# spaceandtimefdn/blitzar

Hardware: NVIDIA H100
Metric: MSM throughput (scalar*point terms/sec), ristretto255, n=2^20 per GPU (higher is better)
Workload: dtype u32 limbs (integer modular arithmetic)

## Files before the change

blitzar_b200/csrc/api.cu:

```cuda
#include <algorithm>
#include <cctype>
#include <cstdint>
#include <cstdio>
#include <cstdlib>
#include <cstring>
#include <condition_variable>
#include <functional>
#include <mutex>
#include <thread>
#include <memory>
#include <string>
#include <vector>

#include "engine_api.cuh"

using namespace b200;

namespace {

struct State {
  bool initialized = false;
  int device = -1;
  cudaStream_t stream = nullptr;
  cudaStream_t copy_stream = nullptr;
// ... 1314 lines not shown
    B200_CUDA(cudaEventDestroy(copied[k]));
  }
}
unsigned b200_multiexp_handle_add_partition_table(struct sxt_multiexp_handle* handle,
                                                  unsigned window_width) {
  const Entry entry("b200_multiexp_handle_add_partition_table");
  return handle_add_partition_table(handle_of(handle), window_width);
}
unsigned b200_multiexp_handle_partition_window(const struct sxt_multiexp_handle* handle) {
  std::lock_guard<std::mutex> lock(g_mutex);
  const HandleSet* hs = handle_of(handle);
  return hs->shards.empty() ? 0u : hs->shards[0]->ptable_w;
}
namespace {
uint64_t check_multi_pairing(unsigned curve_id, const void* out, uint32_t num_products,
                             const uint32_t* lengths, const void* g1, const void* g2) {
  B200_REQUIRE(curve_id == SXT_CURVE_BLS_381 || curve_id == SXT_CURVE_BN_254,
               "pairings are defined for curve ids 1 (bls12-381) and 2 (bn254) only");
  B200_REQUIRE(num_products == 0 || (out != nullptr && lengths != nullptr),
               "out / lengths must not be null");
  uint64_t total = 0;
  for (uint32_t k = 0; k < num_products; ++k)
    total += lengths[k];
  B200_REQUIRE(total < (1ull << 31), "2^31 or more pairs in one call");
  B200_REQUIRE(total == 0 || (g1 != nullptr && g2 != nullptr), "g1 / g2 must not be null");
  return total;
}
}

void b200_multi_pairing(unsigned curve_id, void* out, uint32_t num_products,
                        const uint32_t* lengths, const void* g1, const void* g2) {
  const Entry entry("b200_multi_pairing");
  const uint64_t n = check_multi_pairing(curve_id, out, num_products, lengths, g1, g2);
  if (num_products == 0)
    return;
  cudaStream_t s = g_state.stream;
  const size_t b1 = curve_vtable(curve_id).abi_proj_bytes;
  const size_t b2 = curve_vtable(curve_id == SXT_CURVE_BLS_381 ? B200_CURVE_BLS12_381_G2
                                                               : B200_CURVE_BN254_G2).abi_proj_bytes;
  const size_t gt = curve_id == SXT_CURVE_BLS_381 ? sizeof(b200_bls12_381_gt) : sizeof(b200_bn254_gt);
  DevBuf<unsigned char> d1(n * b1, s), d2(n * b2, s), dout(num_products * gt, s);
  copy_h2d(d1.p, g1, n * b1, s);
  copy_h2d(d2.p, g2, n * b2, s);
  multi_pairing(ctx(), curve_id, dout.p, num_products, lengths, d1.p, d2.p);
  copy_d2h(out, dout.p, num_products * gt, s);
  stream_sync(s);
}
void b200_multi_pairing_device(unsigned curve_id, void* out, uint32_t num_products,
                               const uint32_t* lengths, const void* g1, const void* g2) {
  const Entry entry("b200_multi_pairing_device");
  check_multi_pairing(curve_id, out, num_products, lengths, g1, g2);
  if (num_products == 0)
    return;
  multi_pairing(ctx(), curve_id, out, num_products, lengths, g1, g2);
}
namespace {
void check_points_call(unsigned curve_id, bool pointers_set, uint64_t n) {
  B200_REQUIRE(curve_id >= SXT_CURVE_BLS_381 && curve_id <= B200_CURVE_BN254_G2,
               "point checks are defined for curve ids 1-5 (a ristretto255 encoding is checked by "
               "decoding it)");
  B200_REQUIRE(n == 0 || pointers_set, "valid / points must not be null");
}
uint64_t count_valid(const uint8_t* valid, uint64_t n) {
  uint64_t count = 0;
  for (uint64_t i = 0; i < n; ++i)
    count += valid[i] != 0;
  return count;
}
}

uint64_t b200_check_points(unsigned curve_id, uint8_t* valid, const void* points, uint64_t n) {
  const Entry entry("b200_check_points");
  check_points_call(curve_id, valid != nullptr && points != nullptr, n);
  if (n == 0)
    return 0;
  cudaStream_t s = g_state.stream;
  const size_t bytes = curve_vtable(curve_id).abi_proj_bytes;
  DevBuf<unsigned char> dp(n * bytes, s), dv(n, s);
  copy_h2d(dp.p, points, n * bytes, s);
  check_points(ctx(), curve_id, dv.p, dp.p, n);
  copy_d2h(valid, dv.p, n, s);
  stream_sync(s);
  return count_valid(valid, n);
}
uint64_t b200_decode_points(unsigned curve_id, void* out_p2, uint8_t* valid, const void* encoded,
                            uint64_t n) {
  const Entry entry("b200_decode_points");
  check_points_call(curve_id, out_p2 != nullptr && valid != nullptr && encoded != nullptr, n);
  if (n == 0)
    return 0;
  cudaStream_t s = g_state.stream;
  const CurveVTable& vt = curve_vtable(curve_id);
  DevBuf<unsigned char> de(n * vt.abi_commit_bytes, s), dout(n * vt.abi_proj_bytes, s), dv(n, s);
  copy_h2d(de.p, encoded, n * vt.abi_commit_bytes, s);
  decode_points(ctx(), curve_id, dout.p, dv.p, de.p, n);
  copy_d2h(out_p2, dout.p, n * vt.abi_proj_bytes, s);
  copy_d2h(valid, dv.p, n, s);
  stream_sync(s);
  return count_valid(valid, n);
}
void b200_check_points_device(unsigned curve_id, uint8_t* valid, const void* points, uint64_t n) {
  const Entry entry("b200_check_points_device");
  check_points_call(curve_id, valid != nullptr && points != nullptr, n);
  check_points(ctx(), curve_id, valid, points, n);
}
void b200_decode_points_device(unsigned curve_id, void* out_p2, uint8_t* valid,
                               const void* encoded, uint64_t n) {
  const Entry entry("b200_decode_points_device");
  check_points_call(curve_id, out_p2 != nullptr && valid != nullptr && encoded != nullptr, n);
  decode_points(ctx(), curve_id, out_p2, valid, encoded, n);
}
unsigned b200_selftest_lane_arithmetic(unsigned warps, unsigned seed) {
  const Entry entry("b200_selftest_lane_arithmetic");
  return selftest_lane_arithmetic(ctx(), warps, seed);
}
unsigned b200_field_op(unsigned field, unsigned op, uint64_t n, const uint32_t* a,
                       const uint32_t* b, uint32_t* out) {
  const Entry entry("b200_field_op");
  B200_REQUIRE(n == 0 || (a != nullptr && out != nullptr), "null operand or result array");
  return field_op(ctx(), field, op, n, a, b, out);
}
unsigned b200_selftest_sort(const sxt_sequence_descriptor* columns, unsigned num,
                            unsigned window_bits) {
  const Entry entry("b200_selftest_sort");
  B200_REQUIRE(num == 0 || columns != nullptr, "columns == nullptr");
  B200_REQUIRE(window_bits <= 20, "window_bits in 0..20");
  return selftest_sort(ctx(), columns, num, window_bits);
}
void b200_set_reduce_groups(unsigned g1, unsigned gn) {
  std::lock_guard<std::mutex> lock(g_mutex);
  auto pow2 = [](unsigned v, unsigned dflt) {
    if (v < 2)
      return dflt;
    unsigned p = 2;
    while (p * 2 <= v)
      p *= 2;
    return p;
  };
  g_state.opt.reduce_g1 = pow2(g1, 16u);
  g_state.opt.reduce_gn = pow2(gn, 4u);
}
void b200_profile_accumulate(int enable) {
  std::lock_guard<std::mutex> lock(g_mutex);
  KernelTimer::get().enabled = enable != 0;
}
void b200_profile_read(float* total_ms, unsigned* launches) {
  std::lock_guard<std::mutex> lock(g_mutex);
  KernelTimer::get().read(total_ms, launches);
}
void b200_set_tuning(unsigned window_bits, unsigned chunk1, unsigned chunkn) {
  std::lock_guard<std::mutex> lock(g_mutex);
  g_state.opt.window_bits = window_bits;
  g_state.opt.chunk1 = chunk1;
  g_state.opt.chunkn = chunkn ? chunkn : 8;
}

}
```

blitzar_b200/csrc/engine_api.cuh:

```cuda
#pragma once
#include <algorithm>
#include <cmath>
#include <cstdint>
#include <vector>

#include "../../include/blitzar_b200.h"
#include "runtime.cuh"

namespace b200 {

struct MsmOptions {
  u32 window_bits = 0;
  u32 chunk1 = 0;
  u32 chunkn = 8;
  u32 reduce_g1 = 16;
  u32 reduce_gn = 4;
  u64 quad_threshold = 32768;
  u64 max_group_entries = 1ull << 30;
  u64 max_range_entries = 1ull << 31;
  int pair_levels = -1;
  u32 pair_batch = 0;
  int range_skew = 0;
  u32 uniform_add = 2;
  u32 gens_normalized = 0;
  const u32* unit_veto = nullptr;
  u32 normalize_gens = 1;
  u32 lane_tail = 1;
  u32 scatter_window_major = 0;
  u32 sort_path = 1;
  u32 table_policy = 0;
};

struct EngineCtx {
  stream_t s;
  MsmOptions opt;
  const void* builtin;
  uint64_t num_builtin;
  stream_t tail = stream_t();
  u32 builtin_window_bits = 0, builtin_windows = 0;
  u32 partition_policy = 0;
};

struct Handle {
  unsigned curve_id;
  unsigned n;
  void* gens;
  unsigned window_bits = 0, windows = 1;
  void* ptable = nullptr;
  unsigned ptable_w = 0;
  uint64_t ptable_groups = 0;
};

inline unsigned table_window_bits(uint64_t n, size_t gen_bytes, double budget_bytes) {
  if (n < 1024)
    return 0;
  unsigned best = 0;
  double best_cost = 1e300;
  for (unsigned c = 10; c <= 20; ++c) {
    const double W = 256 / c + 1;
    if (W * (double)n * (double)gen_bytes > budget_bytes || W * (double)n >= 2147483648.0)
      continue;
    const double cost = W * (double)n + 2.5 * (double)(1u << (c - 1));
    if (cost < best_cost) {
      best_cost = cost;
      best = c;
    }
  }
  return best;
}

template <class T> struct DevBuf {
  T* p = nullptr;
  stream_t s;
  DevBuf(size_t count, stream_t s_) : s(s_) { p = (T*)dev_alloc(count * sizeof(T), s); }
  ~DevBuf() { dev_free(p, s); }
  DevBuf(const DevBuf&) = delete;
  DevBuf& operator=(const DevBuf&) = delete;
};

inline uint64_t range_begin(uint64_t n, uint32_t r, uint32_t num_ranges, int skew = 0) {
  if (r == 0)
    return 0;
  if (r >= num_ranges)
    return n;
  if (skew == 0 || n < 64ull * num_ranges)
    return n * r / num_ranges;
  const double t = (double)r / (double)num_ranges;
  const double f = skew > 0 ? 1.0 - (1.0 - t) * std::sqrt(1.0 - t) : t * std::sqrt(t);
  uint64_t b = (uint64_t)((double)n * f);
  const uint64_t lo = r, hi = n - (num_ranges - r);
  return b < lo ? lo : (b > hi ? hi : b);
}
typedef void (*range_wait_fn)(void* user, uint64_t begin, uint64_t end);

inline uint64_t check_descriptors(const sxt_sequence_descriptor* d, uint32_t num) {
  B200_REQUIRE(d != nullptr, "descriptors == nullptr");
  uint64_t longest = 0;
  for (uint32_t i = 0; i < num; ++i) {
    B200_REQUIRE(d[i].n == 0 || d[i].data != nullptr, "descriptor.n > 0 with data == nullptr");
    B200_REQUIRE(d[i].element_nbytes != 0 && d[i].element_nbytes <= 32,
                 "descriptor.element_nbytes must be in 1..32");
    if (d[i].is_signed)
      B200_REQUIRE(d[i].element_nbytes <= 16 &&
                       (d[i].element_nbytes & (d[i].element_nbytes - 1)) == 0,
                   "signed columns need a power-of-two element_nbytes <= 16");
    B200_REQUIRE(d[i].n < (1ull << 31), "column too long");
    longest = longest < d[i].n ? d[i].n : longest;
  }
  return longest;
}

inline uint64_t fixed_row_bytes(int mode, unsigned element_num_bytes, const unsigned* bit_table,
                                unsigned num_outputs) {
  uint64_t row_bits = 0;
  if (mode == 0) {
    B200_REQUIRE(element_num_bytes >= 1 && element_num_bytes <= 32, "element_num_bytes in 1..32");
    row_bits = 8ull * element_num_bytes * num_outputs;
  } else {
    for (unsigned j = 0; j < num_outputs; ++j) {
      B200_REQUIRE(bit_table[j] > 0 && bit_table[j] <= 256, "output bit width must be in 1..256");
      row_bits += bit_table[j];
    }
  }
  return (row_bits + 7) / 8;
}

struct GenLayout {
  struct Piece {
    uint64_t src, pos, count;
  };
  std::vector<Piece> segments;
  std::vector<uint32_t> base;
  uint64_t total = 0;
  uint64_t max_n = 0;

  GenLayout(const sxt_sequence_descriptor* d, uint32_t num, const uint64_t* offsets)
      : base(num, 0), n_(num, 0) {
    std::vector<uint32_t> order;
    for (uint32_t j = 0; j < num; ++j) {
      n_[j] = d[j].n;
      max_n = std::max<uint64_t>(max_n, d[j].n);
      if (d[j].n) {
        B200_REQUIRE(offset(offsets, j) <= ~0ull - d[j].n, "generator offset + column length overflows");
        order.push_back(j);
      }
    }
    std::stable_sort(order.begin(), order.end(), [offsets](uint32_t a, uint32_t b) {
      return offset(offsets, a) < offset(offsets, b);
    });
    for (uint32_t j : order) {
      const uint64_t lo = offset(offsets, j), hi = lo + n_[j];
      if (segments.empty() || lo > segments.back().src + segments.back().count) {
        const uint64_t pos = segments.empty() ? 0 : segments.back().pos + segments.back().count;
        segments.push_back({lo, pos, 0});
      }
      Piece& s = segments.back();
      s.count = std::max(s.count, hi - s.src);
      B200_REQUIRE(s.pos + s.count < (1ull << 31),
                   "merged generator intervals of 2^31 or more generators");
      base[j] = (uint32_t)(s.pos + (lo - s.src));
    }
    total = segments.empty() ? 0 : segments.back().pos + segments.back().count;
  }
  bool within(uint64_t limit) const {
    return segments.empty() || segments.back().src + segments.back().count <= limit;
  }
  std::vector<Piece> needed(uint64_t b, uint64_t e) const {
// ... 177 lines not shown
```

blitzar_b200/csrc/msm.cuh:

```cuda
#pragma once
#include <algorithm>
#include <vector>

#include "batch_affine.cuh"
#include "curve.cuh"
#include "engine_api.cuh"
#include "lanefield.cuh"

namespace b200 {

struct ColumnDesc {
  const unsigned char* base;
  u64 row_stride;
  u32 bit_offset;
  u32 bit_width;
  u32 n;
  u32 is_signed;
  u32 first_window;
  u32 num_windows;
  u32 table_n;
  u32 gen_base;
};
B200_HD u32 bucket_windows(const ColumnDesc& col) { return col.table_n ? (col.num_windows ? 1u : 0u) : col.num_windows; }

// ... 383 lines not shown
    __syncthreads();
    for (u32 i = threadIdx.x; i < size; i += kBlock) {
      const u64 e = stage[i];
      tmp[delta[__ldg(&map[entry_key(e) >> sh])] + i] = e;
    }
  }
};

struct BinSortBody {
  static constexpr int kBlock = 1024;
  static constexpr size_t kSmem = kBinCap * sizeof(u64) + kBinSpan * sizeof(u32);
  const u64* tmp;
  const u32* bin_start;
  const u32* bin_micro;
  const u32* nbins_ptr;
  u32 shift;
  u64 nkeys;
  u64* entries;
  u32* counts;
  __device__ void run(u32 b, unsigned char* smem) const {
    __shared__ u32 ws[32];
    if (b >= *nbins_ptr)
      return;
    u64* sorted = (u64*)smem;
    u32* h = (u32*)(smem + kBinCap * sizeof(u64));
    const u32 lo = bin_start[b], size = bin_start[b + 1] - lo;
    const u64 klo = (u64)bin_micro[b] << shift, khi_m = (u64)bin_micro[b + 1] << shift;
    const u32 span = (u32)((khi_m < nkeys ? khi_m : nkeys) - klo);
    const bool local = size <= kBinCap;
    for (u32 k = threadIdx.x; k < span; k += kBlock)
      h[k] = 0;
    __syncthreads();
#pragma unroll 4
    for (u32 i = threadIdx.x; i < size; i += kBlock)
      atomicAdd(&h[entry_key(tmp[(u64)lo + i]) - (u32)klo], 1u);
    __syncthreads();
    const u32 per = (span + kBlock - 1) / kBlock, k0 = min(threadIdx.x * per, span),
              k1 = min(k0 + per, span);
    u32 sum = 0;
    for (u32 k = k0; k < k1; ++k)
      sum += h[k];
    u32 total;
    u32 run = block_exclusive_scan<kBlock>(sum, ws, &total);
    for (u32 k = k0; k < k1; ++k) {
      const u32 n = h[k];
      h[k] = run;
      run += n;
      counts[klo + k] = lo + run;
    }
    __syncthreads();
    if (!local) {
      for (u32 i = threadIdx.x; i < size; i += kBlock) {
        const u64 e = tmp[(u64)lo + i];
        entries[(u64)lo + atomicAdd(&h[entry_key(e) - (u32)klo], 1u)] = e;
      }
      return;
    }
#pragma unroll 4
    for (u32 i = threadIdx.x; i < size; i += kBlock) {
      const u64 e = tmp[(u64)lo + i];
      sorted[atomicAdd(&h[entry_key(e) - (u32)klo], 1u)] = e;
    }
    __syncthreads();
    for (u32 i = threadIdx.x; i < size; i += kBlock)
      entries[(u64)lo + i] = sorted[i];
  }
};

inline u32 binned_sort_shift(u64 nkeys) {
  u32 shift = 0;
  while ((nkeys + (1ull << shift) - 1) >> shift > kMicroBins)
    ++shift;
  return shift;
}

inline void binned_sort(stream_t s, const ColumnDesc* d_cols, const u64* d_col_start, u32 ncols,
                        u32 c, u32 nbuckets, u64 total_terms, u64 max_entries, u32 max_windows,
                        u64 nkeys, u64* entries, u32* counts, u32* d_m) {
  const u32 shift = binned_sort_shift(nkeys);
  const u32 nmicro = (u32)((nkeys + (1ull << shift) - 1) >> shift);
  const u32 span_micro = std::max(1u, kBinSpan >> shift);
  u32* ws = (u32*)dev_alloc((5ull * nmicro + 3) * sizeof(u32), s);
  u32 *micro_counts = ws, *bin_of = ws + nmicro, *bin_cursor = ws + 2ull * nmicro,
      *bin_start = ws + 3ull * nmicro, *bin_micro = ws + 4ull * nmicro + 1,
      *nbins = ws + 5ull * nmicro + 2;
  u64* tmp = (u64*)dev_alloc(std::max<u64>(max_entries, 1) * sizeof(u64), s);
  dev_zero(micro_counts, nmicro * sizeof(u32), s);
  const u64 count_tile = 4096;
  launch_blocks(MicroCountBody{d_cols, d_col_start, ncols, c, nbuckets, total_terms,
                               (u32)count_tile, shift, nmicro, micro_counts},
                (total_terms + count_tile - 1) / count_tile, nmicro * sizeof(u32), s);
  launch_blocks(PlanBinsBody{micro_counts, nmicro, span_micro, nkeys, bin_of, bin_start, bin_micro,
                             bin_cursor, nbins, counts, d_m},
                1, nmicro * sizeof(u32), s);
  const size_t scatter_smem = 220 * 1024;
  const size_t bin_bytes = (2ull * nmicro + 2) * sizeof(u32);
  const u64 stage_entries = (scatter_smem - bin_bytes) / sizeof(u64);
  u64 scatter_tile = std::max<u64>(1, stage_entries / max_windows);
  if (scatter_tile > (u64)CoarseScatterBody::kBlock)
    scatter_tile -= scatter_tile % CoarseScatterBody::kBlock;
  launch_blocks(CoarseScatterBody{d_cols, d_col_start, ncols, c, nbuckets, total_terms,
                                  (u32)scatter_tile, shift, nmicro, bin_of, nbins, bin_cursor, tmp},
                (total_terms + scatter_tile - 1) / scatter_tile, scatter_smem, s);
  launch_blocks(BinSortBody{tmp, bin_start, bin_micro, nbins, shift, nkeys, entries, counts}, nmicro,
                BinSortBody::kSmem, s);
  dev_free(tmp, s);
  dev_free(ws, s);
}
#endif

template <class C> struct FillIdentityBody {
  static constexpr int kBlock = 256;
  static constexpr u32 kChunks = sizeof(typename C::Point) / 16;
  static_assert(sizeof(typename C::Point) % 16 == 0, "points are made of 16-byte aligned fields");
  uint4* p;
  B200_HD void operator()(u64 t) const {
    const typename C::Point id = C::identity();
    const u32 k = (u32)(t % kChunks);
    uint4 v = ((const uint4*)&id)[0];
#pragma unroll
    for (u32 j = 1; j < kChunks; ++j)
      if (j == k)
        v = ((const uint4*)&id)[j];
    p[t] = v;
  }
};
template <class C> inline void fill_identity(stream_t s, typename C::Point* p, u64 n) {
  launch(FillIdentityBody<C>{(uint4*)p}, n * FillIdentityBody<C>::kChunks, s);
}

struct BucketOffsets {
  const u32* ends;
  const u32* starts;
  B200_HD u32 begin(u64 k) const { return starts ? starts[k] : (k ? ends[k - 1] : 0u); }
  B200_HD u32 end(u64 k) const { return ends[k]; }
};

template <class C> struct MergeBucketsBody {
  static constexpr int kBlock = 128;
  BucketOffsets offsets;
  const typename C::Point* scratch;
  typename C::Point* buckets;
  B200_HD void operator()(u64 k) const {
    if (offsets.begin(k) == offsets.end(k))
      return;
    typename C::Point b = buckets[k];
    C::add(b, b, scratch[k]);
    buckets[k] = b;
  }
};

template <class C, bool kGather, class X = SeqExec, bool kUniform = false, bool kUnitZ = false>
struct AccumulateBody {
  static constexpr int kBlock = 128;
  static constexpr int kMinBlocks = !kGather ? 1 : (C::F::N > 8 ? 2 : 3);
  typedef typename C::Point Point;
  typedef typename C::Gen Gen;
  const u32* keys;
  const u64* entries;
  const Gen* gens;
  const Point* pieces;
  const u32* m_ptr;
  u32 K;
  u32 final_level;
  Point* buckets;
  u32* out_keys;
  Point* out_pieces;
  u32* out_m_ptr;
  const u32* unit_veto;

  B200_HD void close_run(u64 t, u32 key, const Point& acc, bool writer, bool& first_seg) const {
    if (final_level || !first_seg) {
      if (writer)
        buckets[key] = acc;
    } else if (writer) {
      out_keys[2 * t] = key;
      out_pieces[2 * t] = acc;
    }
    first_seg = false;
  }
  template <bool kUnit> B200_HD Gen load_gen(u32 idx) const {
    if constexpr (kUnit)
      return C::load_unit_gen(gens + idx);
    else
      return gens[idx];
  }
  template <bool kUnit>
  B200_HD void gather_walk(u64 t, u64 b, u64 e, bool writer, u32& cur, Point& acc,
                           bool& first_seg) const {
    u64 ent = entries[b];
    Gen g = load_gen<kUnit>(entry_gen(ent));
    cur = entry_key(ent);
    for (u64 i = b; i < e; ++i) {
      u64 ent_n = ent;
      Gen g_n = g;
      if (i + 1 < e) {
        ent_n = entries[i + 1];
        g_n = load_gen<kUnit>(entry_gen(ent_n));
      }
      const u32 k = entry_key(ent);
      const bool negate = entry_negate(ent);
      if (kUniform) {
        if (i == b || k != cur) {
          if (i != b) {
            close_run(t, cur, acc, writer, first_seg);
            cur = k;
          }
          acc = C::identity();
        }
        C::template add_gen<X>(acc, acc, g, negate, kUnit);
      } else {
        const bool start = i == b || k != cur;
        if (k != cur) {
          close_run(t, cur, acc, writer, first_seg);
          cur = k;
        }
        if (start)
          C::gen_to_point(acc, g, negate);
        else
          C::template add_gen<X>(acc, acc, g, negate, kUnit);
      }
      ent = ent_n;
      g = g_n;
    }
  }
  B200_HD void operator()(u64 tid) const {
    const u64 t = tid / X::kLanes;
    const bool writer = (tid % X::kLanes) == 0;
    const u64 M = *m_ptr;
    const u64 T = (M + K - 1) / K;
    if (tid == 0 && out_m_ptr)
      *out_m_ptr = final_level ? 0u : (u32)(2 * T);
    u64 b = t * K;
    if (b >= M)
      return;
    u64 e = b + K < M ? b + K : M;
    u32 cur;
    Point acc;
    bool first_seg = true;
    if constexpr (kGather) {
      if (kUnitZ && unit_veto && *unit_veto)
        gather_walk<false>(t, b, e, writer, cur, acc, first_seg);
      else
        gather_walk<kUnitZ>(t, b, e, writer, cur, acc, first_seg);
    } else {
      cur = keys[b];
      acc = pieces[b];
      for (u64 i = b + 1; i < e; ++i) {
        const u32 k = keys[i];
        if (k == cur) {
          C::template add<X>(acc, acc, pieces[i]);
        } else {
          close_run(t, cur, acc, writer, first_seg);
          cur = k;
          acc = pieces[i];
        }
      }
    }
    if (final_level) {
      close_run(t, cur, acc, writer, first_seg);
      return;
    }
    if (!writer)
      return;
    if (first_seg) {
      close_run(t, cur, acc, writer, first_seg);
      acc = C::identity();
    }
    out_keys[2 * t + 1] = cur;
    out_pieces[2 * t + 1] = acc;
  }
};

struct WindowUsedBody {
  static constexpr int kBlock = 64;
  BucketOffsets offsets;
  u32 nbuckets;
  u32* window_used;
  B200_HD void operator()(u64 w) const {
    if (offsets.begin(w * nbuckets) != offsets.begin((w + 1) * nbuckets))
      window_used[w] = 1u;
  }
};

template <class C, class Ex = SeqExec> struct ReduceBody {
  static constexpr int kBlock = 64;
  typedef typename C::Point Point;
  const Point* X;
  const Point* Cin;
  u32 m_in, g, log2g;
  Point* Xout;
  Point* Cout;
  const u32* window_used;
  u32 nbuckets;
  B200_HD void operator()(u64 tid) const {
    const u64 t = tid / Ex::kLanes;
    const bool writer = (tid % Ex::kLanes) == 0;
    const u32 m_out = m_in / g;
    const u32 w = (u32)(t / m_out), k = (u32)(t % m_out);
    if (window_used[w] == 0) {
      if (writer) {
        Xout[t] = C::identity();
        Cout[t] = C::identity();
      }
      return;
    }
    const Point* x = X + (u64)w * m_in + (u64)k * g;
    Point run = x[g - 1];
    Point acc = Cin ? C::identity() : run;
    if (Cin) {
      acc = run;
      if (g == 1)
        acc = C::identity();
    }
    for (u32 r = g - 1; r-- > 0;) {
      C::template add<Ex>(run, run, x[r]);
      if (r > 0 || !Cin)
        C::template add<Ex>(acc, acc, run);
    }
    if (Cin) {
      const Point* cin = Cin + (u64)w * m_in + (u64)k * g;
      for (u32 r = 0; r < g; ++r)
        C::template add<Ex>(acc, acc, cin[r]);
    }
    for (u32 i = 0; i < log2g; ++i)
      C::template dbl<Ex>(run, run);
    if (writer) {
      Xout[t] = run;
      Cout[t] = acc;
    }
  }
};

template <class C, class X = SeqExec> struct CombineBody {
  static constexpr int kBlock = 32;
  typedef typename C::Point Point;
  const Point* S;
  const ColumnDesc* cols;
  u32 c;
  Point* out;
  B200_HD void operator()(u64 tid) const {
    const u64 j = tid / X::kLanes;
    const bool writer = (tid % X::kLanes) == 0;
    const ColumnDesc col = cols[j];
    if (col.num_windows == 0 || col.n == 0) {
      if (writer)
        out[j] = C::identity();
      return;
    }
    const u32 nw = bucket_windows(col);
    Point acc = S[col.first_window + nw - 1];
    for (u32 w = nw - 1; w-- > 0;) {
      for (u32 i = 0; i < c; ++i)
        C::template dbl<X>(acc, acc);
      C::template add<X>(acc, acc, S[col.first_window + w]);
    }
    if (writer)
      out[j] = acc;
  }
};

#if defined(__CUDACC__) && !defined(B200_EMULATE)
#define B200_LANE_TAIL 1
struct CombineLaneBody {
  static constexpr int kBlock = 32;
  typedef Ed25519 C;
  const C::Point* S;
  const ColumnDesc* cols;
  u32 c;
  C::Point* out;
  __device__ void operator()(u64 tid) const {
    const u64 j = tid >> 5;
    const ColumnDesc col = cols[j];
    if (col.num_windows == 0 || col.n == 0) {
      if ((tid & 31u) == 0)
        out[j] = C::identity();
      return;
    }
    const lane10::Lane L = lane10::lane_info();
    const u32 nw = bucket_windows(col);
    C::Point acc = S[col.first_window + nw - 1];
    for (u32 w = nw - 1; w-- > 0;) {
      u32 t;
      const u32 v = lane10::dbl_n(L, lane10::slice_point(L, acc), (int)c, t);
      lane10::gather_point(acc, v, t);
      C::add<QuadExecConv>(acc, acc, S[col.first_window + w]);
    }
    if ((tid & 31u) == 0)
      out[j] = acc;
  }
};
struct LanePow {
  static __device__ __forceinline__ void pow22523(F25519::E& r, const F25519::E& a) {
    const lane10::Lane L = lane10::lane_info();
    const u32 g = L.base / 10u;
    lane10::gather(r, lane10::pow22523(L, lane10::slice(L, a)), g < 3 ? g : 0u);
  }
};
struct StoreLaneBody {
  static constexpr int kBlock = 32;
  const Ed25519::Point* pts;
  unsigned char* out;
  u64 count;
  __device__ void operator()(u64 tid) const {
    const u32 lane = (u32)tid & 31u, g = lane / 10u;
    const u64 i = (tid >> 5) * 3 + g;
    const bool live = g < 3 && i < count;
    unsigned char enc[32];
    Ed25519::encode<LanePow>(enc, pts[live ? i : count - 1]);
    if (live && lane == 10u * g) {
      uint4* d = (uint4*)(out + 32 * i);
      const uint4* e = (const uint4*)enc;
      d[0] = e[0];
      d[1] = e[1];
    }
  }
};
#endif

template <class C>
inline void launch_store_commit(stream_t s, const typename C::Point* pts, unsigned char* out,
                                u64 count, bool lane_tail = true);

template <class C, bool kProjective> struct IngestBody {
  static constexpr int kBlock = 128;
// ... 395 lines not shown
  p.c = opt.window_bits ? opt.window_bits
                        : choose_window_bits(p.max_n, max_width, p.ncols, point_bytes);
  p.nbuckets = 1u << (p.c - 1);
  u64 max_entries = 0;
  for (auto& col : cols) {
    col.first_window = p.total_windows;
    col.num_windows = col.n ? col.bit_width / p.c + 1 : 0;
    p.total_windows += bucket_windows(col);
    max_entries += (u64)col.n * col.num_windows;
    if (col.table_n)
      B200_REQUIRE((u64)col.table_n * col.num_windows < (1ull << 31), "generator table too large");
    if (col.n)
      B200_REQUIRE((u64)col.gen_base + col.n + (u64)(col.num_windows - 1) * col.table_n < (1ull << 31),
                   "generator index of a column too large");
  }
  p.nkeys = (u64)p.total_windows * p.nbuckets;
  p.total_entries = max_entries;
  B200_REQUIRE(p.nkeys < (1ull << 32), "too many buckets for one pass");
  p.cols = std::move(cols);
  return p;
}

struct StagedRange {
  const ColumnDesc* d_cols = nullptr;
  const u64* d_col_start = nullptr;
  u64 total_terms = 0, max_entries = 0;
  u32 max_windows = 0;
  StagedRange(stream_t s, const MsmPlan& plan, u64 begin, u64 end) {
    const u32 ncols = plan.ncols;
    std::vector<ColumnDesc> cols(plan.cols);
    std::vector<u64> col_start(ncols + 1, 0);
    for (u32 j = 0; j < ncols; ++j) {
      u64 lo = std::min<u64>(begin, cols[j].n), hi = std::min<u64>(end, cols[j].n);
      cols[j].base += lo * cols[j].row_stride;
      cols[j].n = (u32)(hi - lo);
      col_start[j + 1] = col_start[j] + cols[j].n;
      max_entries += (u64)cols[j].n * cols[j].num_windows;
      max_windows = std::max(max_windows, cols[j].n ? cols[j].num_windows : 0u);
    }
    total_terms = col_start[ncols];
    if (total_terms == 0)
      return;
    B200_REQUIRE(max_entries < (1ull << 32) && end - begin < (1ull << 31),
                 "too many (term, window) entries for one sort pass");
    const size_t desc_bytes = ncols * sizeof(ColumnDesc), start_bytes = (ncols + 1) * sizeof(u64);
    std::vector<unsigned char> stage(desc_bytes + start_bytes);
    std::memcpy(stage.data(), cols.data(), desc_bytes);
    std::memcpy(stage.data() + desc_bytes, col_start.data(), start_bytes);
    d_cols = (const ColumnDesc*)stage_to_device(s, stage.data(), stage.size());
    d_col_start = (const u64*)((const unsigned char*)d_cols + desc_bytes);
  }
};

struct SortedLayout {
  u64* entries;
  u32* counts;
  u32* starts;
  u32* d_m;
  u64 slots_max;
  bool binned;
  BucketOffsets offsets() const { return {counts, starts}; }
};

inline SortedLayout sort_entries(stream_t s, const MsmPlan& plan, const StagedRange& r, u32 L,
                                 const MsmOptions& opt, u32* window_used) {
  const u32 ncols = plan.ncols, c = plan.c, nbuckets = plan.nbuckets;
  const u64 nkeys = plan.nkeys, max_entries = r.max_entries, total_terms = r.total_terms;
  SortedLayout out{};
  out.slots_max = L ? ((max_entries + nkeys * ((1ull << L) - 1) + (1ull << L) - 1) >> L) << L : max_entries;
  out.counts = (u32*)dev_alloc((nkeys + 1) * sizeof(u32), s);
  out.d_m = (u32*)dev_alloc(16 * sizeof(u32), s);
  out.entries = (u64*)dev_alloc(out.slots_max * sizeof(u64), s);
#ifdef B200_BINNED_SORT
  out.binned = L == 0 && opt.sort_path != 0 && binned_sort_shift(nkeys) <= kMaxBinShift &&
               (opt.sort_path == 2 || max_entries >= kBinnedSortMinEntries);
  if (out.binned)
    binned_sort(s, r.d_cols, r.d_col_start, ncols, c, nbuckets, total_terms, max_entries,
                r.max_windows, nkeys, out.entries, out.counts, out.d_m);
#endif
  if (!out.binned) {
    dev_zero(out.counts, (nkeys + 1) * sizeof(u32), s);
    launch(CountBody{r.d_cols, r.d_col_start, ncols, c, nbuckets, out.counts}, total_terms, s);
    if (L)
      launch(PadCountsBody{out.counts, (1u << L) - 1u}, nkeys, s);
    exclusive_scan(out.counts, nkeys + 1, s);
    copy_d2d(out.d_m, out.counts + nkeys, sizeof(u32), s);
    if (L) {
      out.starts = (u32*)dev_alloc((nkeys + 1) * sizeof(u32), s);
      copy_d2d(out.starts, out.counts, (nkeys + 1) * sizeof(u32), s);
    }
    const bool window_major = opt.scatter_window_major && r.max_windows > 1;
    launch(ScatterBody{r.d_cols, r.d_col_start, ncols, c, nbuckets, out.counts, out.entries,
                       window_major ? total_terms : 0},
           window_major ? total_terms * r.max_windows : total_terms, s);
  }
  if (L)
    launch(FillPadsBody{out.starts, out.counts, out.entries}, nkeys, s);
  launch(WindowUsedBody{out.offsets(), nbuckets, window_used}, plan.total_windows, s);
  return out;
}

inline unsigned sort_selftest(stream_t s, std::vector<ColumnDesc> cols, u32 c) {
  MsmOptions opt;
  opt.window_bits = c;
  const MsmPlan plan = msm_make_plan(std::move(cols), opt, 160);
  const StagedRange r(s, plan, 0, plan.max_n);
  if (r.total_terms == 0)
    return ~0u;
  const u64 nkeys = plan.nkeys, M = r.max_entries;
  DevBuf<u32> window_used(plan.total_windows, s);
  opt.sort_path = 0;
  const SortedLayout a = sort_entries(s, plan, r, 0, opt, window_used.p);
  opt.sort_path = 2;
  const SortedLayout b = sort_entries(s, plan, r, 0, opt, window_used.p);
  std::vector<u32> ca(nkeys + 1), cb(nkeys + 1), m(1);
  std::vector<u64> ea(M), eb(M);
  copy_d2h(ca.data(), a.counts, (nkeys + 1) * sizeof(u32), s);
  copy_d2h(cb.data(), b.counts, (nkeys + 1) * sizeof(u32), s);
  copy_d2h(m.data(), b.d_m, sizeof(u32), s);
  copy_d2h(ea.data(), a.entries, M * sizeof(u64), s);
  copy_d2h(eb.data(), b.entries, M * sizeof(u64), s);
  stream_sync(s);
  for (void* p : {(void*)a.entries, (void*)a.counts, (void*)a.d_m, (void*)b.entries, (void*)b.counts,
                  (void*)b.d_m, (void*)r.d_cols})
    dev_free(p, s);
  if (!b.binned)
    return ~0u;
  unsigned bad = m[0] == ca[nkeys] ? 0u : 1u;
  for (u64 k = 0; k < nkeys; ++k) {
    const u32 lo = k ? ca[k - 1] : 0u, hi = ca[k];
    if (cb[k] != hi || hi < lo || hi > M) {
      ++bad;
      continue;
    }
    std::sort(ea.begin() + lo, ea.begin() + hi);
    std::sort(eb.begin() + lo, eb.begin() + hi);
    if (!std::equal(ea.begin() + lo, ea.begin() + hi, eb.begin() + lo))
      ++bad;
  }
  return bad;
}

struct RangeHook {
  virtual void before_range(u64 begin, u64 end) = 0;
  virtual void before_accumulate() {}
  virtual ~RangeHook() {}
};

template <class C>
stream_t chunk_walk(stream_t s, stream_t tail, WalkInput<C> walk, u32* d_m, bool unit,
                    const u32* unit_veto, typename C::Point* target, const MsmOptions& opt,
                    std::vector<void*>& to_free) {
  typedef typename C::Point Point;
  u32 K = opt.chunk1 ? std::max(opt.chunk1, 4u) : (walk.m_max >= (1ull << 23) ? 64u : 32u);
  const u32 chunkn = std::max(opt.chunkn, 4u);
  const u32* lvl_keys = nullptr;
  const Point* lvl_pieces = nullptr;
  stream_t cs = s;
  for (int level = 0;; ++level) {
    const bool final_level = walk.m_max <= K;
    u64 T = (walk.m_max + K - 1) / K;
    u32* out_keys = final_level ? nullptr : (u32*)dev_alloc(2 * T * sizeof(u32), cs);
    Point* out_pieces = final_level ? nullptr : (Point*)dev_alloc(2 * T * sizeof(Point), cs);
    to_free.insert(to_free.end(), {out_keys, out_pieces});
    u32* out_m = d_m + 1 + (level % 8);
    const auto launch_level = [&](auto body, u64 threads, stream_t st) {
      body = {lvl_keys, walk.entries, walk.gens, lvl_pieces, walk.m_ptr, K, final_level, target,
              out_keys, out_pieces, out_m, unit_veto};
      launch(body, threads, st);
    };
    if (level == 0) {
      const bool uniform =
          opt.uniform_add == 2 ? C::kCurveId == kRistretto255 : opt.uniform_add != 0;
      constexpr bool kEd = C::kCurveId == kRistretto255;
      const bool unit_path = kEd && unit;
      if (uniform && unit_path)
        launch_level(AccumulateBody<C, true, SeqExec, true, kEd>{}, T, s);
      else if (uniform)
        launch_level(AccumulateBody<C, true, SeqExec, true>{}, T, s);
      else if (unit_path)
        launch_level(AccumulateBody<C, true, SeqExec, false, kEd>{}, T, s);
      else
        launch_level(AccumulateBody<C, true>{}, T, s);
      KernelTimer::get().end(s);
      if (tail != s)
        stream_follow(tail, s);
      cs = tail;
    } else if (T <= opt.quad_threshold) {
      launch_level(AccumulateBody<C, false, QuadExec>{}, T * QuadExec::kLanes, cs);
    } else {
      launch_level(AccumulateBody<C, false>{}, T, cs);
    }
    if (final_level)
      break;
    lvl_keys = out_keys;
    lvl_pieces = out_pieces;
    walk.m_ptr = out_m;
    walk.m_max = 2 * T;
    K = chunkn;
  }
  return cs;
}

template <class C>
void msm_accumulate_range(stream_t s, const MsmPlan& plan, const typename C::Gen* gens, u64 begin,
                          u64 end, bool add_into, typename C::Point* d_buckets,
                          u32* d_window_used, const MsmOptions& opt, stream_t tail,
                          RangeHook* hook = nullptr) {
  const StagedRange r(s, plan, begin, end);
  if (r.total_terms == 0)
    return;
  gens += begin;
  StageRange nvtx_sort("msm: digit count + scan + scatter");
  const u64 max_entries = r.max_entries, nkeys = plan.nkeys;
  u32 L = 0;
  if constexpr (C::kBatchAffine) {
    const double mean = (double)max_entries / (double)nkeys;
    if (opt.pair_levels >= 0)
      L = (u32)opt.pair_levels;
    else if (max_entries >= (1ull << 23))
      while (L < 6 && (double)(32u << L) <= mean)
        ++L;
    while (L > 0 && max_entries + nkeys * ((1ull << L) - 1) >= (1ull << 32) - (1ull << L))
      --L;
  }
  const SortedLayout sorted = sort_entries(s, plan, r, L, opt, d_window_used);
  B200_LOG(3, "range [%llu, %llu): %llu terms, %llu entries max, c=%u, %llu keys, pair levels %u",
           (unsigned long long)begin, (unsigned long long)end, (unsigned long long)r.total_terms,
           (unsigned long long)max_entries, plan.c, (unsigned long long)nkeys, L);
  WalkInput<C> walk{gens, sorted.entries, sorted.d_m, max_entries};
  std::vector<void*> to_free;
  if (hook)
    hook->before_accumulate();
  KernelTimer::get().begin(s);
  StageRange nvtx_acc("msm: bucket accumulation");
  if constexpr (C::kBatchAffine) {
    if (L) {
      walk = run_pair_levels<C>(s, L, sorted.entries, gens, sorted.d_m, sorted.slots_max,
                                opt.pair_batch);
      to_free = {(void*)walk.gens, (void*)walk.entries};
    }
  }
  typedef typename C::Point Point;
  Point* target = add_into ? (Point*)dev_alloc(nkeys * sizeof(Point), s) : d_buckets;
  const bool unit = walk.gens == gens && opt.gens_normalized;
  const stream_t cs =
      chunk_walk<C>(s, tail, walk, sorted.d_m, unit, opt.unit_veto, target, opt, to_free);
  if (add_into) {
    launch(MergeBucketsBody<C>{sorted.offsets(), target, d_buckets}, nkeys, cs);
    dev_free(target, cs);
  }
  to_free.insert(to_free.end(), {sorted.d_m, sorted.counts, sorted.starts});
  for (void* ptr : to_free)
    dev_free(ptr, cs);
  dev_free(sorted.entries, s);
  dev_free((void*)r.d_cols, s);
}

template <class C>
void msm_finish(stream_t s, const MsmPlan& plan, const typename C::Point* d_buckets,
                const u32* d_window_used, typename C::Point* out, const MsmOptions& opt) {
  typedef typename C::Point Point;
  StageRange nvtx_fin("msm: bucket reduction + window combination");
  const u32 total_windows = plan.total_windows, nbuckets = plan.nbuckets, ncols = plan.ncols;
  ColumnDesc* d_cols =
      (ColumnDesc*)stage_to_device(s, plan.cols.data(), ncols * sizeof(ColumnDesc));
  Point* d_S = nullptr;
  u32 m = nbuckets;
  const Point* X = d_buckets;
  const Point* Cin = nullptr;
  std::vector<void*> to_free;
  if (m == 1) {
    d_S = (Point*)dev_alloc(total_windows * sizeof(Point), s);
    copy_d2d(d_S, d_buckets, total_windows * sizeof(Point), s);
  }
  bool first = true;
  while (m > 1) {
    u32 g = first ? std::min<u32>(opt.reduce_g1, m) : std::min<u32>(opt.reduce_gn, m);
    u32 log2g = 0;
    while ((1u << log2g) < g)
      ++log2g;
    u32 m_out = m / g;
    Point* Xout = (Point*)dev_alloc((u64)total_windows * m_out * sizeof(Point), s);
    Point* Cout = (Point*)dev_alloc((u64)total_windows * m_out * sizeof(Point), s);
    if ((u64)total_windows * m_out <= opt.quad_threshold)
      launch(ReduceBody<C, QuadExecConv>{X, Cin, m, g, log2g, Xout, Cout, d_window_used, nbuckets},
             (u64)total_windows * m_out * QuadExec::kLanes, s);
    else
      launch(ReduceBody<C>{X, Cin, m, g, log2g, Xout, Cout, d_window_used, nbuckets},
             (u64)total_windows * m_out, s);
    to_free.push_back(Xout);
    if (m_out > 1)
      to_free.push_back(Cout);
    X = Xout;
    Cin = Cout;
    m = m_out;
    first = false;
    if (m == 1)
      d_S = Cout;
  }
  for (void* ptr : to_free)
    dev_free(ptr, s);
  bool uniform_windows = true;
  for (u32 j = 1; j < ncols; ++j)
    uniform_windows = uniform_windows && bucket_windows(plan.cols[j]) == bucket_windows(plan.cols[0]);
#ifdef B200_LANE_TAIL
  bool lane_done = false;
  if constexpr (C::kCurveId == kRistretto255) {
    if (ncols <= 2048 && opt.lane_tail) {
      launch(CombineLaneBody{d_S, d_cols, plan.c, out}, (u64)ncols * 32, s);
      lane_done = true;
    }
  }
  if (lane_done) {
  } else
#endif
  if (ncols <= opt.quad_threshold && uniform_windows)
    launch(CombineBody<C, QuadExecConv>{d_S, d_cols, plan.c, out}, (u64)ncols * QuadExec::kLanes,
           s);
  else if (ncols <= opt.quad_threshold)
    launch(CombineBody<C, QuadExec>{d_S, d_cols, plan.c, out}, (u64)ncols * QuadExec::kLanes, s);
  else
    launch(CombineBody<C>{d_S, d_cols, plan.c, out}, ncols, s);
  dev_free(d_S, s);
  dev_free(d_cols, s);
}

template <class C>
void msm_run(stream_t s, const typename C::Gen* gens, std::vector<ColumnDesc> cols,
             typename C::Point* out, const MsmOptions& opt = MsmOptions(), u32 num_ranges = 1,
             RangeHook* hook = nullptr, stream_t tail = stream_t()) {
  typedef typename C::Point Point;
  if (cols.empty())
    return;
  MsmPlan plan = msm_make_plan(std::move(cols), opt, sizeof(Point));
  B200_LOG(2, "msm: curve %u, %u columns, longest %llu, %llu terms, window %u bits, %u bucket sets%s",
           C::kCurveId, plan.ncols, (unsigned long long)plan.max_n,
           (unsigned long long)plan.total_terms, plan.c, plan.total_windows,
           plan.ncols && plan.cols[0].table_n ? " (fixed-base table)" : "");
  if (plan.total_terms == 0 || plan.total_windows == 0) {
    if (hook)
      hook->before_range(0, plan.max_n);
    fill_identity<C>(s, out, plan.ncols);
    return;
  }
  Point* d_buckets = (Point*)dev_alloc(plan.nkeys * sizeof(Point), s);
  fill_identity<C>(s, d_buckets, plan.nkeys);
  u32* d_window_used = (u32*)dev_alloc(plan.total_windows * sizeof(u32), s);
  dev_zero(d_window_used, plan.total_windows * sizeof(u32), s);
  if (num_ranges < 1)
    num_ranges = 1;
  const u64 limit = opt.max_range_entries ? opt.max_range_entries : (1ull << 31);
  const u64 needed = (plan.total_entries + limit - 1) / limit;
  if (needed > num_ranges)
// ... 19 lines not shown
```

Measured before the change: 368.3 million.

## Replace multi-level piece accumulation with single-pass segment merge and tree reduction

After the first gather-accumulate level, the repeated chunked accumulate levels are replaced by two kernels. MergeShortBody sums short bucket runs directly. Long runs are recorded through an atomic counter, and MergeLongBody reduces them with an in-place S-ary tree that uses arrival counters and fences. This removes per-level launches and intermediate allocations, at the cost of atomics, L2-bypassing loads and extra complexity. The default chunkn drops from 8 to 4.

```diff
diff --git a/blitzar_b200/csrc/api.cu b/blitzar_b200/csrc/api.cu
--- a/blitzar_b200/csrc/api.cu
+++ b/blitzar_b200/csrc/api.cu
@@ -1490,7 +1490,7 @@
   std::lock_guard<std::mutex> lock(g_mutex);
   g_state.opt.window_bits = window_bits;
   g_state.opt.chunk1 = chunk1;
-  g_state.opt.chunkn = chunkn ? chunkn : 8;
-}
-
-}
+  g_state.opt.chunkn = chunkn ? chunkn : MsmOptions().chunkn;
+}
+
+}
diff --git a/blitzar_b200/csrc/engine_api.cuh b/blitzar_b200/csrc/engine_api.cuh
--- a/blitzar_b200/csrc/engine_api.cuh
+++ b/blitzar_b200/csrc/engine_api.cuh
@@ -12,7 +12,7 @@
 struct MsmOptions {
   u32 window_bits = 0;
   u32 chunk1 = 0;
-  u32 chunkn = 8;
+  u32 chunkn = 4;
   u32 reduce_g1 = 16;
   u32 reduce_gn = 4;
   u64 quad_threshold = 32768;
diff --git a/blitzar_b200/csrc/msm.cuh b/blitzar_b200/csrc/msm.cuh
--- a/blitzar_b200/csrc/msm.cuh
+++ b/blitzar_b200/csrc/msm.cuh
@@ -559,14 +559,13 @@
 
 template <class C, bool kGather, class X = SeqExec, bool kUniform = false, bool kUnitZ = false>
 struct AccumulateBody {
+  static_assert(kGather, "pieces are summed by MergeShortBody / MergeLongBody");
   static constexpr int kBlock = 128;
-  static constexpr int kMinBlocks = !kGather ? 1 : (C::F::N > 8 ? 2 : 3);
+  static constexpr int kMinBlocks = C::F::N > 8 ? 2 : 3;
   typedef typename C::Point Point;
   typedef typename C::Gen Gen;
-  const u32* keys;
   const u64* entries;
   const Gen* gens;
-  const Point* pieces;
   const u32* m_ptr;
   u32 K;
   u32 final_level;
@@ -645,25 +644,10 @@
     u32 cur;
     Point acc;
     bool first_seg = true;
-    if constexpr (kGather) {
-      if (kUnitZ && unit_veto && *unit_veto)
-        gather_walk<false>(t, b, e, writer, cur, acc, first_seg);
-      else
-        gather_walk<kUnitZ>(t, b, e, writer, cur, acc, first_seg);
-    } else {
-      cur = keys[b];
-      acc = pieces[b];
-      for (u64 i = b + 1; i < e; ++i) {
-        const u32 k = keys[i];
-        if (k == cur) {
-          C::template add<X>(acc, acc, pieces[i]);
-        } else {
-          close_run(t, cur, acc, writer, first_seg);
-          cur = k;
-          acc = pieces[i];
-        }
-      }
-    }
+    if (kUnitZ && unit_veto && *unit_veto)
+      gather_walk<false>(t, b, e, writer, cur, acc, first_seg);
+    else
+      gather_walk<kUnitZ>(t, b, e, writer, cur, acc, first_seg);
     if (final_level) {
       close_run(t, cur, acc, writer, first_seg);
       return;
@@ -678,6 +662,142 @@
     out_pieces[2 * t + 1] = acc;
   }
 };
+
+struct LongSegment {
+  u32 start, end;
+  u32 leaf0;
+  u32 key;
+};
+struct MergeScratch {
+  unsigned long long* counter;
+  u32* arrivals;
+  LongSegment* segs;
+};
+
+B200_HD void device_fence() {
+#ifdef __CUDA_ARCH__
+  __threadfence();
+#endif
+}
+template <class T> B200_HD T load_l2(const T* p) {
+#ifdef __CUDA_ARCH__
+  static_assert(sizeof(T) % 16 == 0, "points are made of 16-byte aligned fields");
+  union {
+    T v;
+    uint4 q[sizeof(T) / 16];
+  } u;
+#pragma unroll
+  for (u32 k = 0; k < sizeof(T) / 16; ++k)
+    u.q[k] = __ldcg((const uint4*)p + k);
+  return u.v;
+#else
+  return *p;
+#endif
+}
+
+template <class C> struct MergeShortBody {
+  static constexpr int kBlock = 128;
+  typedef typename C::Point Point;
+  const u32* keys;
+  const Point* pieces;
+  const u32* m_ptr;
+  u32 S;
+  Point* buckets;
+  MergeScratch scratch;
+  B200_HD void operator()(u64 t) const {
+    const u32 m = *m_ptr, i0 = (u32)(2 * t);
+    if (i0 >= m)
+      return;
+    const u32 k0 = keys[i0];
+    const bool start0 = i0 == 0 || keys[i0 - 1] != k0;
+    const bool start1 = i0 + 1 < m && keys[i0 + 1] != k0;
+    if (start0 && start1)
+      buckets[k0] = pieces[i0];
+    if (!start1 && !start0)
+      return;
+    const u32 i = start1 ? i0 + 1 : i0, key = keys[i];
+    u32 e = i + 1;
+    while (e < m && e - i <= S && keys[e] == key)
+      ++e;
+    if (e - i <= S) {
+      Point acc = pieces[i];
+      for (u32 j = i + 1; j < e; ++j)
+        C::add(acc, acc, pieces[j]);
+      buckets[key] = acc;
+      return;
+    }
+    u32 hi = m;
+    while (e < hi) {
+      const u32 mid = e + (hi - e) / 2;
+      if (keys[mid] == key)
+        e = mid + 1;
+      else
+        hi = mid;
+    }
+    const u32 leaves = (e - i + S - 1) / S;
+    const unsigned long long slot =
+        B200_ATOMIC_ADD(scratch.counter, ((unsigned long long)leaves << 32) | 1ull);
+    scratch.segs[(u32)slot] = LongSegment{i, e, (u32)(slot >> 32), key};
+  }
+};
+
+template <class C> struct MergeLongBody {
+  static constexpr int kBlock = 128;
+  typedef typename C::Point Point;
+  Point* pieces;
+  u32 S;
+  Point* buckets;
+  MergeScratch scratch;
+  B200_HD void operator()(u64 g) const {
+    const unsigned long long count = *scratch.counter;
+    const u32 nsegs = (u32)count;
+    if (g >= (count >> 32))
+      return;
+    u32 lo = 0, hi = nsegs - 1;
+    while (lo < hi) {
+      const u32 mid = lo + (hi - lo + 1) / 2;
+      if (scratch.segs[mid].leaf0 <= g)
+        lo = mid;
+      else
+        hi = mid - 1;
+    }
+    const LongSegment seg = scratch.segs[lo];
+    Point* p = pieces + seg.start;
+    const u64 len = seg.end - seg.start;
+    Point acc;
+    u64 j = (g - seg.leaf0) * S;
+    for (u64 w = 1; w < len; w *= S, j /= S) {
+      const u64 first = j / S * S * w, left = (len - first + w - 1) / w, kids = left < S ? left : S;
+      if (w > 1) {
+        if (kids == 1)
+          continue;
+        p[j * w] = acc;
+        device_fence();
+        if (B200_ATOMIC_ADD(&scratch.arrivals[seg.leaf0 + (first + w) / S], 1u) != kids - 1)
+          return;
+        device_fence();
+      }
+      acc = load_l2(p + first);
+      for (u64 k = 1; k < kids; ++k)
+        C::add(acc, acc, load_l2(p + first + k * w));
+    }
+    buckets[seg.key] = acc;
+  }
+};
+
+template <class C>
+void merge_pieces(stream_t s, const u32* keys, typename C::Point* pieces, const u32* m_ptr,
+                  u64 m_max, u32 S, typename C::Point* buckets, std::vector<void*>& to_free) {
+  const u64 seg_max = m_max / (S + 1) + 1, leaf_max = m_max / S + seg_max;
+  const size_t head = sizeof(unsigned long long) + leaf_max * sizeof(u32);
+  unsigned char* mem = (unsigned char*)dev_alloc(head + seg_max * sizeof(LongSegment), s);
+  dev_zero(mem, head, s);
+  const MergeScratch scratch{(unsigned long long*)mem, (u32*)(mem + sizeof(unsigned long long)),
+                             (LongSegment*)(mem + head)};
+  launch(MergeShortBody<C>{keys, pieces, m_ptr, S, buckets, scratch}, (m_max + 1) / 2, s);
+  launch(MergeLongBody<C>{pieces, S, buckets, scratch}, leaf_max, s);
+  to_free.push_back(mem);
+}
 
 struct WindowUsedBody {
   static constexpr int kBlock = 64;
@@ -1379,54 +1499,35 @@
                     const u32* unit_veto, typename C::Point* target, const MsmOptions& opt,
                     std::vector<void*>& to_free) {
   typedef typename C::Point Point;
-  u32 K = opt.chunk1 ? std::max(opt.chunk1, 4u) : (walk.m_max >= (1ull << 23) ? 64u : 32u);
-  const u32 chunkn = std::max(opt.chunkn, 4u);
-  const u32* lvl_keys = nullptr;
-  const Point* lvl_pieces = nullptr;
-  stream_t cs = s;
-  for (int level = 0;; ++level) {
-    const bool final_level = walk.m_max <= K;
-    u64 T = (walk.m_max + K - 1) / K;
-    u32* out_keys = final_level ? nullptr : (u32*)dev_alloc(2 * T * sizeof(u32), cs);
-    Point* out_pieces = final_level ? nullptr : (Point*)dev_alloc(2 * T * sizeof(Point), cs);
-    to_free.insert(to_free.end(), {out_keys, out_pieces});
-    u32* out_m = d_m + 1 + (level % 8);
-    const auto launch_level = [&](auto body, u64 threads, stream_t st) {
-      body = {lvl_keys, walk.entries, walk.gens, lvl_pieces, walk.m_ptr, K, final_level, target,
-              out_keys, out_pieces, out_m, unit_veto};
-      launch(body, threads, st);
-    };
-    if (level == 0) {
-      const bool uniform =
-          opt.uniform_add == 2 ? C::kCurveId == kRistretto255 : opt.uniform_add != 0;
-      constexpr bool kEd = C::kCurveId == kRistretto255;
-      const bool unit_path = kEd && unit;
-      if (uniform && unit_path)
-        launch_level(AccumulateBody<C, true, SeqExec, true, kEd>{}, T, s);
-      else if (uniform)
-        launch_level(AccumulateBody<C, true, SeqExec, true>{}, T, s);
-      else if (unit_path)
-        launch_level(AccumulateBody<C, true, SeqExec, false, kEd>{}, T, s);
-      else
-        launch_level(AccumulateBody<C, true>{}, T, s);
-      KernelTimer::get().end(s);
-      if (tail != s)
-        stream_follow(tail, s);
-      cs = tail;
-    } else if (T <= opt.quad_threshold) {
-      launch_level(AccumulateBody<C, false, QuadExec>{}, T * QuadExec::kLanes, cs);
-    } else {
-      launch_level(AccumulateBody<C, false>{}, T, cs);
-    }
-    if (final_level)
-      break;
-    lvl_keys = out_keys;
-    lvl_pieces = out_pieces;
-    walk.m_ptr = out_m;
-    walk.m_max = 2 * T;
-    K = chunkn;
-  }
-  return cs;
+  const u32 K = opt.chunk1 ? opt.chunk1 : (walk.m_max >= (1ull << 23) ? 64u : 32u);
+  const bool final_level = walk.m_max <= K;
+  const u64 T = (walk.m_max + K - 1) / K;
+  u32* keys = final_level ? nullptr : (u32*)dev_alloc(2 * T * sizeof(u32), s);
+  Point* pieces = final_level ? nullptr : (Point*)dev_alloc(2 * T * sizeof(Point), s);
+  to_free.insert(to_free.end(), {keys, pieces});
+  u32* m_pieces = d_m + 1;
+  const auto launch_level = [&](auto body) {
+    body = {walk.entries, walk.gens, walk.m_ptr, K, final_level, target, keys, pieces, m_pieces,
+            unit_veto};
+    launch(body, T, s);
+  };
+  const bool uniform = opt.uniform_add == 2 ? C::kCurveId == kRistretto255 : opt.uniform_add != 0;
+  constexpr bool kEd = C::kCurveId == kRistretto255;
+  const bool unit_path = kEd && unit;
+  if (uniform && unit_path)
+    launch_level(AccumulateBody<C, true, SeqExec, true, kEd>{});
+  else if (uniform)
+    launch_level(AccumulateBody<C, true, SeqExec, true>{});
+  else if (unit_path)
+    launch_level(AccumulateBody<C, true, SeqExec, false, kEd>{});
+  else
+    launch_level(AccumulateBody<C, true>{});
+  KernelTimer::get().end(s);
+  if (tail != s)
+    stream_follow(tail, s);
+  if (!final_level)
+    merge_pieces<C>(tail, keys, pieces, m_pieces, 2 * T, std::max(opt.chunkn, 2u), target, to_free);
+  return tail;
 }
 
 template <class C>
```

Result: faster. 378.4 million (median of 6 runs) (+2.7%).
